# mjmyt/drone_path_planning_python

Measured on AMD Instinct MI355X. Metric: minimum-snap trajectories/sec (N drones × M segments, order 7) at 1/2/4/8 MI355X, higher is better.
Workload: dtype f64

## Files before the change

drone_path_planning_python_amd/csrc/msnap_collide.hip:

```cpp
#include <math.h>

#include "msnap_internal.h"
#include "msnap_collide.h"
#include "msnap_wave.h"

namespace msnap {


struct CollideGeom {
  int R, ro, Cn, S;
  int Rp;
  int os, oe;
  int sym;
  int n_rb;
  int upw;
  int upw_tail;
  long long split;
  int sparts;
  long long total;
  long long u_lo, u_n;
  int I_lo, I_hi;
  int part;
};

// ... 396 lines not shown
        bv[u] = e < nG * 6 ? cu.colbox[e] : 0.0;
      }
#pragma unroll
      for (int u = 0; u < kStageGroups * 6 / kSelThreads; ++u) {
        const int e = threadIdx.x + u * kSelThreads;
        if (e < nG * 6) sBox[e] = bv[u];
      }
    }
    __syncthreads();
  }
  auto load_box = [&](int gq, double(&B)[6]) {
#pragma unroll
    for (int k = 0; k < 6; ++k) {
      if constexpr (kStage) B[k] = sBox[gq * 6 + k];
      else B[k] = cu.colbox[(size_t)gq * 6 + k];
    }
  };
  if ((int)blockIdx.x >= n_rb) {
    constexpr int NW = kSelThreads / kWave, NS = kSelGroups * kSelTrips;
    __shared__ int gsum[NS * NW + 1];
    __shared__ int gbase, gtot;
    const int a0 = (blockIdx.x - n_rb) * kSelGroups, nG = (N + kColBlock - 1) / kColBlock;
    const int lane = threadIdx.x & (kWave - 1), w = threadIdx.x / kWave;
    unsigned long long kept = 0;
#pragma unroll
    for (int ai = 0; ai < kSelGroups; ++ai) {
      const int a = a0 + ai;
      double A[7], A6[6];
      load_box(a < nG ? a : nG - 1, A6);
#pragma unroll
      for (int k = 0; k < 6; ++k) A[k] = A6[k];
      A[6] = sCmax[a < nG ? a : nG - 1];
#pragma unroll
      for (int t = 0; t < kSelTrips; ++t) {
        bool keep = false;
        if (a + t * kSelThreads < nG) {
          const int b = a + t * kSelThreads + threadIdx.x, bc = b < nG ? b : nG - 1;
          double B6[6];
          load_box(bc, B6);
          const double lb2 = box_box_lb2(A, B6);
          keep = b < nG && (b == a || !((lb2 > A[6]) & (lb2 > sCmax[bc])));
        }
        const unsigned long long m = __ballot(keep);
        kept |= keep ? 1ull << (ai * kSelTrips + t) : 0ull;
        if (lane == 0) gsum[(ai * kSelTrips + t) * NW + w] = __popcll(m);
      }
    }
    __syncthreads();
    if (threadIdx.x < kWave) {
      int run = 0;
      for (int i0 = 0; i0 < NS * NW; i0 += kWave) {
        const int v = i0 + lane < NS * NW ? gsum[i0 + lane] : 0;
        int inc = v;
#pragma unroll
        for (int m = 1; m < kWave; m <<= 1) {
          const int o = __shfl_up(inc, m);
          inc += lane >= m ? o : 0;
        }
        if (i0 + lane < NS * NW) gsum[i0 + lane] = run + inc - v;
        run += __shfl(inc, kWave - 1);
      }
      if (lane == 0) {
        gbase = atomicAdd(&meta[kMetaGroups], run);
        gtot = run;
      }
    }
    __syncthreads();
    if (threadIdx.x < kSelGroups && a0 + (int)threadIdx.x < nG) {
      const int ai = threadIdx.x;
      const int s0 = gsum[ai * kSelTrips * NW], s1 = ai + 1 < kSelGroups ? gsum[(ai + 1) * kSelTrips * NW] : gtot;
      cg.astart[a0 + ai] = gbase + s0;
      cg.acnt[a0 + ai] = s1 - s0;
    }
#pragma unroll
    for (int ai = 0; ai < kSelGroups; ++ai)
#pragma unroll
      for (int t = 0; t < kSelTrips; ++t) {
        const bool keep = (kept >> (ai * kSelTrips + t)) & 1ull;
        const unsigned long long m = __ballot(keep);
        const int pos = gbase + gsum[(ai * kSelTrips + t) * NW + w] + __popcll(m & ((1ull << lane) - 1ull));
        if (keep && pos < cg.cap) {
          const int a = a0 + ai, b = a + t * kSelThreads + threadIdx.x;
          cg.glist[pos] = (a << 16) | b;
          if (b != a) cg.blist[(size_t)b * cg.nG + a] = pos + 1;
        }
      }
    return;
  }
  constexpr int GPB = kRowBlock / kColBlock;
  constexpr int NW = kSelThreads / kWave;
  __shared__ int wsum[kSelTrips][NW];
  __shared__ int sStart;
  __shared__ double sRow[GPB][8];
  __shared__ double sAll[8];
  const int I = blockIdx.x, lane = threadIdx.x & (kWave - 1), w = threadIdx.x / kWave;
  const int nsh = (N - I * kRowBlock + kColBlock - 1) / kColBlock;
  const int ng = nsh < GPB ? nsh : GPB;
  if (threadIdx.x < 7 * GPB) {
    const int q = threadIdx.x / 7, k = threadIdx.x % 7;
    if (q < ng) sRow[q][k] = k < 6 ? (kStage ? sBox[(I * GPB + q) * 6 + k] : cu.colbox[(size_t)(I * GPB + q) * 6 + k]) : sCmax[I * GPB + q];
  }
  __syncthreads();
  if (threadIdx.x < 7) {
    const int k = threadIdx.x;
    double v = sRow[0][k];
    for (int q = 1; q < ng; ++q) v = k < 3 ? fmin(v, sRow[q][k]) : fmax(v, sRow[q][k]);
    sAll[k] = v;
  }
  __syncthreads();
  unsigned long long mk[kSelTrips];
  bool keep[kSelTrips];
  double cbx[kSelTrips][6], cmx[kSelTrips];
#pragma unroll
  for (int t = 0; t < kSelTrips; ++t) {
    if (t * kSelThreads >= nsh) continue;
    const int k = t * kSelThreads + threadIdx.x, J = I * GPB + (k < nsh ? k : nsh - 1);
    load_box(J, cbx[t]);
    cmx[t] = sCmax[J];
  }
#pragma unroll
  for (int t = 0; t < kSelTrips; ++t) {
    const int k = t * kSelThreads + threadIdx.x;
    keep[t] = false;
    if (k < nsh) {
      keep[t] = true;
      if (k >= GPB) {
        const double cm = cmx[t];
        bool any = false;
        const double lb0 = box_box_lb2(sAll, cbx[t]);
        if (!((lb0 > sAll[6]) & (lb0 > cm))) {
          for (int q = 0; q < ng; ++q) {
            const double lb2 = box_box_lb2(sRow[q], cbx[t]);
            any |= !((lb2 > sRow[q][6]) & (lb2 > cm));
          }
        }
        keep[t] = any;
      }
    }
    mk[t] = __ballot(keep[t]);
    if (lane == 0) wsum[t][w] = __popcll(mk[t]);
  }
  __syncthreads();
  int all = 0, off[kSelTrips];
#pragma unroll
  for (int t = 0; t < kSelTrips; ++t) {
#pragma unroll
    for (int q = 0; q < NW; ++q) {
      if (q == w) off[t] = all;
      all += wsum[t][q];
    }
  }
  if (threadIdx.x == 0) {
    const int start = atomicAdd(&meta[kMetaTotal], all);
    sStart = start;
    meta[kMetaStart + I] = start;
    cnt[I] = all;
  }
  __syncthreads();
#pragma unroll
  for (int t = 0; t < kSelTrips; ++t)
    if (keep[t]) list[sStart + off[t] + __popcll(mk[t] & ((1ull << lane) - 1ull))] = (I << 16) | (t * kSelThreads + threadIdx.x);
}

__device__ __forceinline__ void
collide_span_list_body(const double *__restrict__ prow_t, const double *__restrict__ pcol, CollideGeom g,
                       double *__restrict__ part_d2, int32_t *__restrict__ part_j, double *__restrict__ cpart_d2,
                       int32_t *__restrict__ cpart_i, const int32_t *__restrict__ oid, const int32_t *__restrict__ list,
                       int sp_force, int slots, int32_t *__restrict__ meta) {
  constexpr int CB = kColBlock;
  __shared__ double sFold[CB * kWave];
  __shared__ int sFoldI[CB * kWave];
  const int lane = threadIdx.x;
  const int tot = meta[kMetaTotal];
  const CullSplit sp = cull_split(tot, slots, cull_nch(g.S), sp_force);
  if (blockIdx.x == 0 && lane == 0) {
    meta[kMetaParts] = sp.lo;
    meta[kMetaParts + 1] = sp.hi;
    meta[kMetaParts + 2] = sp.x;
  }
  const int items = sp.items(tot);
  const int xi = sp.x * sp.hi;
  auto share_of = [&](int it) { return it < xi ? it / sp.hi : sp.x + (it - xi) / sp.lo; };
  int it = blockIdx.x;
  int entry = it < items ? list[share_of(it)] : 0;
  while (it < items) {
    const int f = share_of(it);
    g.sparts = it < xi ? sp.hi : sp.lo;
    const int h = it - sp.item_of(f);
    const int I = entry >> 16, k = entry & 0xffff;
    const int nxt = it + gridDim.x;
    entry = nxt < items ? list[share_of(nxt)] : 0;
    const int crow = I * sp.hi + h;
    const int cj = I * kRowBlock + k * CB;
    const int ncols = g.Cn - cj < CB ? g.Cn - cj : CB;
    const bool two_sided = k >= kRowBlock / CB;
    RowSet rs;
#pragma unroll
    for (int rr = 0; rr < kRowsPerLane; ++rr) {
      const int raw = I * kRowBlock + rr * kWave + lane;
      rs.live[rr] = raw < g.R;
      rs.grow[rr] = rs.live[rr] ? raw : g.R - 1;
      rs.best[rr] = INFINITY;
      rs.bestj[rr] = -1;
    }
    const double *prowT = prow_t + (size_t)I * kRowBlock;
    if (ncols <= 2)
      collide_block<2, true>(g, prowT, pcol, cj, ncols, two_sided, rs, I, h, crow, lane, sFold, sFoldI, cpart_d2, cpart_i, oid);
    else if (ncols <= CB / 2)
      collide_block<CB / 2, true>(g, prowT, pcol, cj, ncols, two_sided, rs, I, h, crow, lane, sFold, sFoldI, cpart_d2, cpart_i, oid);
    else
      collide_block<CB, true>(g, prowT, pcol, cj, ncols, two_sided, rs, I, h, crow, lane, sFold, sFoldI, cpart_d2, cpart_i, oid);
#pragma unroll
    for (int rr = 0; rr < kRowsPerLane; ++rr) {
      part_d2[(size_t)it * kRowBlock + rr * kWave + lane] = rs.best[rr];
      part_j[(size_t)it * kRowBlock + rr * kWave + lane] = (rs.best[rr] == INFINITY) ? -1 : rs.bestj[rr];
    }
    it = nxt;
  }
}

constexpr int kGroupHalf = kColBlock / 2;
constexpr int kGroupLanes = kWave / 2;

constexpr int kFinishWaves = 4;
template <int kChunks>
__global__ void __launch_bounds__(kWave * kFinishWaves)
collide_finish_groups_kernel(int N, const int32_t *__restrict__ oid, const int32_t *__restrict__ meta, CullGroups cg,
                             double radius, double *__restrict__ min_dist, int32_t *__restrict__ partner,
                             int32_t *__restrict__ hit) {
  __shared__ int sItAll[kFinishWaves][kChunks * kWave];
  const int lane = threadIdx.x & (kWave - 1), w = __builtin_amdgcn_readfirstlane(threadIdx.x / kWave);
  int *sIt = sItAll[w];
  const int gq = blockIdx.x * kFinishWaves + w;
  if (gq >= cg.nG) return;
  int pl[kChunks];
#pragma unroll
  for (int c = 0; c < kChunks; ++c)
    pl[c] = (c * kWave < gq && c * kWave + lane < gq) ? cg.blist[(size_t)gq * cg.nG + c * kWave + lane] : 0;
  if (meta[kMetaGroups] > cg.cap) {
#pragma unroll
    for (int c = 0; c < kChunks; ++c)
      if (pl[c] > 0) cg.blist[(size_t)gq * cg.nG + c * kWave + lane] = 0;
    return;
  }
  const int nA = cg.acnt[gq], sA = cg.astart[gq];
  const int k = lane & (kColBlock - 1), e = lane >> 3;
  const int r = gq * kColBlock + k;
  const int out = r < N ? oid[r] : 0;
  int nB = 0;
#pragma unroll
  for (int c = 0; c < kChunks; ++c) {
    const unsigned long long m = __ballot(pl[c] > 0);
    if (pl[c] > 0) sIt[nB + __popcll(m & ((1ull << lane) - 1ull))] = pl[c] - 1;
    nB += __popcll(m);
  }
  __builtin_amdgcn_fence(__ATOMIC_RELEASE, "wavefront", "local");
  __builtin_amdgcn_wave_barrier();
  __builtin_amdgcn_fence(__ATOMIC_ACQUIRE, "wavefront", "local");
  double best = INFINITY;
  int bj = -1;
  constexpr int U = 8;
  for (int q0 = 0; q0 < nA + nB; q0 += U * (kWave / kColBlock)) {
    double d[U];
    int j[U];
#pragma unroll
    for (int u = 0; u < U; ++u) {
      const int q = q0 + u * (kWave / kColBlock) + e;
      d[u] = INFINITY;
      j[u] = -1;
      if (q < nA + nB) {
        const size_t slot = (q < nA ? (size_t)(sA + q) * 16 : (size_t)sIt[q - nA] * 16 + kColBlock) + k;
        d[u] = cg.cand_d2[slot];
        j[u] = cg.cand_j[slot];
      }
    }
#pragma unroll
    for (int u = 0; u < U; ++u)
      if (j[u] >= 0 && (bj < 0 || d[u] < best || (d[u] == best && j[u] < bj))) {
        best = d[u];
        bj = j[u];
      }
  }
#pragma unroll
  for (int m = kColBlock; m < kWave; m <<= 1) {
    const double o = shfl_xor_f64(best, m);
    const int oj = __shfl_xor(bj, m);
    if (oj >= 0 && (bj < 0 || o < best || (o == best && oj < bj))) {
      best = o;
      bj = oj;
    }
  }
  if (e == 0 && r < N) {
    const double dist = sqrt(bj >= 0 ? best : INFINITY);
    min_dist[out] = dist;
    partner[out] = bj;
    hit[out] = (dist < 2.0 * radius) ? 1 : 0;
  }
#pragma unroll
  for (int c = 0; c < kChunks; ++c)
    if (pl[c] > 0) cg.blist[(size_t)gq * cg.nG + c * kWave + lane] = 0;
}

constexpr int kGroupWaves = 4;
__global__ void __launch_bounds__(kWave, kGroupWaves)
collide_eval_groups_kernel(const double *__restrict__ pcol, int N, int S, const int32_t *__restrict__ oid,
                           const int32_t *__restrict__ meta, CullGroups cg, unsigned long long *__restrict__ hint) {
#pragma clang fp contract(off)
  const int lane = threadIdx.x;
  int tot = meta[kMetaGroups];
  if (blockIdx.x == 0 && lane == 0 && hint != nullptr)
    __hip_atomic_store(hint, cull_hint_pack(N, meta[kMetaTotal], tot), __ATOMIC_RELAXED, __HIP_MEMORY_SCOPE_SYSTEM);
  if (tot > cg.cap) tot = 0;
  const unsigned stride = (unsigned)S * 3u;
  const int per = (tot + 7) >> 3;
  auto item_of = [&](int v) { return (v >> 3) < per ? (v & 7) * per + (v >> 3) : tot; };
  int v = blockIdx.x, it = item_of(v);
  int entry = (it < tot && it < cg.cap) ? cg.glist[it] : 0;
  for (; (v >> 3) < per; v += gridDim.x, it = item_of(v)) {
    const int it_next = item_of(v + (int)gridDim.x);
    const int ent_raw = entry;
    entry = it_next < tot ? cg.glist[it_next] : 0;
    if (it >= tot) continue;
    const int ent = __builtin_amdgcn_readfirstlane(ent_raw);
    const int a = ent >> 16, b = ent & 0xffff;
    const bool diag = a == b;

    int lane_s = threadIdx.x;
    asm volatile("" : "+v"(lane_s));
    const int half = lane_s >> 5, ls = lane_s & (kGroupLanes - 1);
    double acc[kColBlock * kGroupHalf];
#pragma unroll
    for (int p = 0; p < kColBlock * kGroupHalf; ++p) acc[p] = INFINITY;
#pragma unroll 1
    for (int s0 = 0; s0 < S; s0 += kGroupLanes) {
      const int sq = s0 + ls < S ? s0 + ls : S - 1;
      const unsigned voff = (unsigned)sq * 24u;
      double cx[kGroupHalf], cy[kGroupHalf], cz[kGroupHalf];
#pragma unroll
      for (int c = 0; c < kGroupHalf; ++c) {
        const int d = b * kColBlock + half * kGroupHalf + c;
        const double *p = reinterpret_cast<const double *>(
            reinterpret_cast<const char *>(pcol + (size_t)(d < N ? d : N - 1) * stride) + (size_t)voff);
        cx[c] = p[0];
        cy[c] = p[1];
        cz[c] = p[2];
      }
      double rw[3][3];
      auto fetch = [&](int r, double(&dst)[3]) {
        const int d = a * kColBlock + r;
        const double *p = reinterpret_cast<const double *>(
            reinterpret_cast<const char *>(pcol + (size_t)(d < N ? d : N - 1) * stride) + (size_t)voff);
        dst[0] = p[0];
        dst[1] = p[1];
        dst[2] = p[2];
      };
      fetch(0, rw[0]);
      fetch(1, rw[1]);
#pragma unroll
      for (int r = 0; r < kColBlock; ++r) {
        if (r + 2 < kColBlock) fetch(r + 2, rw[(r + 2) % 3]);
        asm volatile("" ::: "memory");
        const double x = rw[r % 3][0], y = rw[r % 3][1], z = rw[r % 3][2];
#pragma unroll
        for (int c = 0; c < kGroupHalf; ++c) {
          const double dx = cx[c] - x, dy = cy[c] - y, dz = cz[c] - z;
          const double d2 = __builtin_fma(dz, dz, __builtin_fma(dy, dy, dx * dx));
          asm("v_min_f64 %0, %1, %0" : "+v"(acc[r * kGroupHalf + c]) : "v"(d2));
        }
      }
    }
#pragma unroll
    for (int n = 16, m = 16; n >= 1; n >>= 1, m >>= 1) {
      const bool up = (lane_s & m) != 0;
#pragma unroll
      for (int i = 0; i < n; ++i) {
        const double keep = up ? acc[i + n] : acc[i], send = up ? acc[i] : acc[i + n];
        acc[i] = __builtin_fmin(keep, __shfl_xor(send, m));
      }
    }
    double v = acc[0];
    int lane_c = threadIdx.x;
    asm volatile("" : "+v"(lane_c));
    const int pr = (lane_c & (kGroupLanes - 1)) >> 2, pc = lane_c & (kGroupHalf - 1), half_c = lane_c >> 5;
    const int ra = a * kColBlock + pr, cb = b * kColBlock + half_c * kGroupHalf + pc;
    const int oi = oid[ra < N ? ra : N - 1], oj = oid[cb < N ? cb : N - 1];
    if (ra >= N || cb >= N || (diag && ra == cb)) v = INFINITY;
    {
      double w = v;
      int wj = oj;
#pragma unroll
      for (int m = 1; m <= 32; m = (m == 2 ? 32 : m << 1)) {
        const double o = __shfl_xor(w, m);
        const int ojx = __shfl_xor(wj, m);
        const bool take = (o < w) | ((o == w) & (ojx < wj));
        w = take ? o : w;
        wj = take ? ojx : wj;
      }
      if ((lane & 35) == 0) {
        cg.cand_d2[(size_t)it * 16 + pr] = w;
        cg.cand_j[(size_t)it * 16 + pr] = w < INFINITY ? wj : -1;
      }
    }
    {
      double w = v;
      int wi = oi;
#pragma unroll
      for (int m = 4; m <= 16; m <<= 1) {
        const double o = __shfl_xor(w, m);
        const int oix = __shfl_xor(wi, m);
        const bool take = (o < w) | ((o == w) & (oix < wi));
        w = take ? o : w;
        wi = take ? oix : wi;
      }
      if ((lane_c & (kGroupLanes - 1)) < kGroupHalf) {
        const int k = kColBlock + half_c * kGroupHalf + pc;
        cg.cand_d2[(size_t)it * 16 + k] = w;
        cg.cand_j[(size_t)it * 16 + k] = (!diag && w < INFINITY) ? wi : -1;
      }
    }
  }
}

__global__ void __launch_bounds__(kWave, 4)
collide_eval_shares_kernel(const double *__restrict__ prow_t, const double *__restrict__ pcol, CollideGeom g,
                           double *__restrict__ part_d2, int32_t *__restrict__ part_j, double *__restrict__ cpart_d2,
                           int32_t *__restrict__ cpart_i, const int32_t *__restrict__ oid, const int32_t *__restrict__ list,
                           int sp_force, int slots, int32_t *__restrict__ meta, unsigned long long *__restrict__ hint,
                           int groups_cap) {
  if (groups_cap > 0 && meta[kMetaGroups] <= groups_cap) return;
  if (blockIdx.x == 0 && threadIdx.x == 0 && hint != nullptr)
    __hip_atomic_store(hint, cull_hint_pack(g.R, meta[kMetaTotal], meta[kMetaGroups]), __ATOMIC_RELAXED,
                       __HIP_MEMORY_SCOPE_SYSTEM);
  collide_span_list_body(prow_t, pcol, g, part_d2, part_j, cpart_d2, cpart_i, oid, list, sp_force, slots, meta);
}

__global__ void __launch_bounds__(kWave)
collide_short_kernel(const double *__restrict__ prow, const double *__restrict__ pcol, int R, int ro, int Cn, int S,
                     double radius, double *__restrict__ min_dist, int32_t *__restrict__ partner,
                     int32_t *__restrict__ hit, int raw) {
#pragma clang fp contract(off)
  const int r = blockIdx.x * kWave + threadIdx.x;
  if (r >= R) return;
  const int grow = ro + r;
  const double *pr = prow + (size_t)r * S * 3;
  double best = INFINITY;
  int bestj = -1;
  for (int j = 0; j < Cn; ++j) {
    const double *pc = pcol + (size_t)j * S * 3;
    double m = INFINITY;
    for (int sq = 0; sq < S; ++sq) {
      const double dx = pc[(size_t)sq * 3 + 0] - pr[(size_t)sq * 3 + 0];
      const double dy = pc[(size_t)sq * 3 + 1] - pr[(size_t)sq * 3 + 1];
      const double dz = pc[(size_t)sq * 3 + 2] - pr[(size_t)sq * 3 + 2];
      const double d2 = __builtin_fma(dz, dz, __builtin_fma(dy, dy, dx * dx));
      m = __builtin_fmin(d2, m);
    }
    if (j == grow) m = INFINITY;
    if (m < best) {
      best = m;
      bestj = j;
    }
  }
  if (raw) {
    min_dist[r] = best;
    partner[r] = (best == INFINITY) ? -1 : bestj;
    return;
  }
  const double dist = sqrt(best);
  min_dist[r] = dist;
  partner[r] = (best == INFINITY) ? -1 : bestj;
  hit[r] = (dist < 2.0 * radius) ? 1 : 0;
}

constexpr int kMergeRows = 16;
constexpr int kMergeParts = 16;
__global__ void __launch_bounds__(kMergeRows * kMergeParts)
collide_merge_kernel(const double *__restrict__ part_d2, const int32_t *__restrict__ part_j, CollideGeom g,
                     const double *__restrict__ cpart_d2, const int32_t *__restrict__ cpart_i, double radius,
                     double *__restrict__ min_dist, int32_t *__restrict__ partner, int32_t *__restrict__ hit,
                     const int32_t *__restrict__ oid, const int32_t *__restrict__ cnt, const int32_t *__restrict__ meta,
                     int groups_cap = 0) {
  if (groups_cap > 0 && meta[kMetaGroups] <= groups_cap) return;
  __shared__ double sD[kMergeParts][kMergeRows];
  __shared__ int sJ[kMergeParts][kMergeRows];
  const int lr = threadIdx.x & (kMergeRows - 1), q = threadIdx.x / kMergeRows;
  const int r_raw = blockIdx.x * kMergeRows + lr;
  const int r = r_raw < g.R ? r_raw : g.R - 1;
  const int out = oid ? oid[r] : r;
  double best = INFINITY;
  int bj = -1;
  constexpr int U = 8;
  auto sweep = [&](const double *pd, const int32_t *pj, size_t pitch, int n) {
    for (int s0 = q; s0 < n; s0 += U * kMergeParts) {
      double v[U];
      int j[U];
#pragma unroll
      for (int k = 0; k < U; ++k) {
        const int sidx = s0 + k * kMergeParts;
        const int sc = sidx < n ? sidx : n - 1;
        v[k] = pd[(size_t)sc * pitch];
        j[k] = sidx < n ? pj[(size_t)sc * pitch] : -1;
      }
#pragma unroll
      for (int k = 0; k < U; ++k) {
        if (j[k] >= 0 && (v[k] < best || (v[k] == best && j[k] < bj))) {
          best = v[k];
          bj = j[k];
        }
      }
    }
  };
  if (cnt) {
    const int I = __builtin_amdgcn_readfirstlane(r / kRowBlock);
    CullSplit sp;
    sp.lo = meta[kMetaParts];
    sp.hi = meta[kMetaParts + 1];
    sp.x = meta[kMetaParts + 2];
    const int f0 = meta[kMetaStart + I], first_item = sp.item_of(f0), n_items = sp.item_of(f0 + cnt[I]) - first_item;
    const size_t first = (size_t)first_item * kRowBlock + (r - I * kRowBlock);
    sweep(part_d2 + first, part_j + first, kRowBlock, n_items);
    if (I > 0) sweep(cpart_d2 + r, cpart_i + r, (size_t)g.R, I * sp.hi);
  } else if (g.total > 0) {
    const int I = r / kRowBlock;
    long long ua = collide_ustart(g, I), ub = collide_ustart(g, I + 1) - 1;
    ua = ua < g.u_lo ? g.u_lo : ua;
    ub = ub >= g.u_lo + g.u_n ? g.u_lo + g.u_n - 1 : ub;
    if (ub >= ua) {
      const long long wf = collide_share_of(g, ua), wl = collide_share_of(g, ub);
      const size_t first = ((size_t)wf + (I - g.I_lo)) * g.sparts * kRowBlock + (r - I * kRowBlock);
      sweep(part_d2 + first, part_j + first, kRowBlock, (int)(wl - wf + 1) * g.sparts);
    }
    const int Ib = I < g.I_hi + 1 ? I : g.I_hi + 1;
    if (g.sym && Ib > g.I_lo) sweep(cpart_d2 + r, cpart_i + r, (size_t)g.R, (Ib - g.I_lo) * g.sparts);
  }
  sD[q][lr] = best;
  sJ[q][lr] = bj;
  __syncthreads();
  if (q == 0 && r_raw < g.R) {
#pragma unroll
    for (int k = 1; k < kMergeParts; ++k) {
      const double v = sD[k][lr];
      const int j = sJ[k][lr];
      if (j >= 0 && (v < best || (v == best && j < bj))) {
        best = v;
        bj = j;
      }
    }
    if (g.part) {
      min_dist[r] = best;
      partner[r] = bj;
    } else {
      const double dist = sqrt(best);
      min_dist[out] = dist;
      partner[out] = bj;
      hit[out] = (dist < 2.0 * radius) ? 1 : 0;
    }
  }
}

__global__ void __launch_bounds__(256)
collide_finish_kernel(const unsigned char *__restrict__ parts, size_t part_stride, int n_parts, int N, int row_offset,
                      int n_rows, double radius, double *__restrict__ min_dist, int32_t *__restrict__ partner,
                      int32_t *__restrict__ hit) {
  const int i = blockIdx.x * 256 + threadIdx.x;
  if (i >= n_rows) return;
  const int r = row_offset + i;
  double best = INFINITY;
  int bj = -1;
  for (int p = 0; p < n_parts; ++p) {
    const unsigned char *base = parts + (size_t)p * part_stride;
    const double v = reinterpret_cast<const double *>(base)[r];
    const int j = reinterpret_cast<const int32_t *>(base + (size_t)N * sizeof(double))[r];
    if (j >= 0 && (v < best || (v == best && j < bj))) {
      best = v;
      bj = j;
    }
  }
  const double dist = sqrt(best);
  min_dist[i] = dist;
  partner[i] = bj;
  hit[i] = (dist < 2.0 * radius) ? 1 : 0;
}

__global__ void __launch_bounds__(256) collide_part_clear_kernel(double *__restrict__ d2, int32_t *__restrict__ pj, int N) {
  const int i = blockIdx.x * 256 + threadIdx.x;
  if (i < N) {
    d2[i] = INFINITY;
    pj[i] = -1;
  }
}


__global__ void __launch_bounds__(kWave * kKeyDrones)
collide_key_kernel(const double *__restrict__ pos, int N, int S, double *__restrict__ box, unsigned *__restrict__ key) {
  const int lane = threadIdx.x & (kWave - 1);
  const int d = blockIdx.x * kKeyDrones + __builtin_amdgcn_readfirstlane(threadIdx.x / kWave);
  if (d >= N) return;
  const double *p = pos + (size_t)d * S * 3;
  double lo[3] = {INFINITY, INFINITY, INFINITY}, hi[3] = {-INFINITY, -INFINITY, -INFINITY};
  const int E = S * 3;
  for (int e0 = 0; e0 < E; e0 += 3 * kWave) {
#pragma unroll
    for (int q = 0; q < 3; ++q) {
      const int e = e0 + q * kWave + lane;
      const double v = e < E ? p[e] : __builtin_nan("");
      const int k = (lane + q) % 3;
      if (__builtin_isfinite(v)) {
#pragma unroll
        for (int kk = 0; kk < 3; ++kk)
          if (k == kk) {
            lo[kk] = v < lo[kk] ? v : lo[kk];
            hi[kk] = v > hi[kk] ? v : hi[kk];
          }
      }
    }
  }
#pragma unroll
  for (int k = 0; k < 3; ++k) {
    lo[k] = uniform_f64(wave_minmax_f64<false>(lo[k]));
    hi[k] = uniform_f64(wave_minmax_f64<true>(hi[k]));
  }
  if (lane < 3) {
    box[(size_t)d * 6 + lane] = lane == 0 ? lo[0] : lane == 1 ? lo[1] : lo[2];
    box[(size_t)d * 6 + 3 + lane] = lane == 0 ? hi[0] : lane == 1 ? hi[1] : hi[2];
  }
  if (lane == 0) key[d] = drone_sort_key(lo, hi);
}

constexpr int kRankWaves = 16;
constexpr int kRankTile = 16;
template <int kRankKeys>
__global__ void __launch_bounds__(kWave * kRankWaves)
collide_rank_kernel(const unsigned *__restrict__ key, int N, int32_t *__restrict__ perm, const double *__restrict__ box,
                    unsigned long long *__restrict__ bound, int32_t *__restrict__ zero, int n_zero,
                    int32_t *__restrict__ meta) {
  __shared__ int cnt[kRankWaves][kRankTile];
  {
    const int gid = blockIdx.x * (kWave * kRankWaves) + threadIdx.x;
    uniform_for<int>(threadIdx.x, n_zero, gridDim.x * (kWave * kRankWaves), [&](int z) { zero[z] = 0; },
                     blockIdx.x * (kWave * kRankWaves));
    if (gid == 0) {
      meta[kMetaTotal] = 0;
      meta[kMetaGroups] = 0;
    }
  }
  const int lane = threadIdx.x & (kWave - 1), w = __builtin_amdgcn_readfirstlane(threadIdx.x / kWave);
  const int nq = (N + kRankWaves * kWave - 1) / (kRankWaves * kWave);
  const int i0 = blockIdx.x * kRankTile;
  unsigned kraw[kRankKeys];
#pragma unroll
  for (int q = 0; q < kRankKeys; ++q) {
    const int j = (w * nq + q) * kWave + lane;
    kraw[q] = key[(q < nq && j < N) ? j : 0];
  }
  const unsigned ktile = key[i0 + (lane & (kRankTile - 1)) < N ? i0 + (lane & (kRankTile - 1)) : N - 1];
  double bx[6] = {0.0, 0.0, 0.0, 0.0, 0.0, 0.0};
  if (threadIdx.x < kRankTile && i0 + (int)threadIdx.x < N) {
#pragma unroll
    for (int k = 0; k < 6; ++k) bx[k] = box[(size_t)(i0 + threadIdx.x) * 6 + k];
  }
  unsigned long long mine[kRankKeys];
#pragma unroll
  for (int q = 0; q < kRankKeys; ++q) {
    const int j = (w * nq + q) * kWave + lane;
    mine[q] = (q < nq && j < N) ? ((unsigned long long)kraw[q] << 32) | (unsigned)j : ~0ull;
  }
#pragma unroll
  for (int t = 0; t < kRankTile; ++t) {
    const int i = i0 + t < N ? i0 + t : N - 1;
    const unsigned long long ki = ((unsigned long long)(unsigned)__builtin_amdgcn_readlane((int)ktile, t) << 32) | (unsigned)i;
    int c = 0;
#pragma unroll
    for (int q = 0; q < kRankKeys; ++q)
      if (q < nq) c += __popcll(__ballot(mine[q] < ki));
    if (lane == 0) cnt[w][t] = c;
  }
  lds_barrier();
  if (threadIdx.x < kRankTile && i0 + (int)threadIdx.x < N) {
    int r = 0;
#pragma unroll
    for (int q = 0; q < kRankWaves; ++q) r += cnt[q][threadIdx.x];
    const int i = i0 + threadIdx.x;
    perm[r] = i;
    const bool has = (bx[0] <= bx[3]) & (bx[1] <= bx[4]) & (bx[2] <= bx[5]);
    bound[r] = has ? 0x7ff0000000000000ull : 0ull;
  }
}

#ifndef MSNAP_TILE_E
#define MSNAP_TILE_E 15
#endif
constexpr int kTileE = MSNAP_TILE_E, kTileRows = 64, kTileHalo = 4;
constexpr int kTilePitch = kTileE + 1 + (kTileE & 1);
static_assert(kTileE % 3 == 0, "whole samples per tile");
constexpr int kBoxGroups = 32;
__global__ void __launch_bounds__(256)
collide_gather_kernel(const double *__restrict__ pos, int N, int Rp, int E, double *__restrict__ prow_t,
                      double *__restrict__ psorted, const int32_t *__restrict__ perm, unsigned long long *__restrict__ bound,
                      const double *__restrict__ box, double *__restrict__ colbox, int nx, int ny, int n_box,
                      int32_t *__restrict__ fill, size_t fill_n) {
#pragma clang fp contract(off)
  __shared__ double tile[(kTileRows + kTileHalo) * kTilePitch];
  __shared__ double sF[kTileHalo][kTileRows];
  const int tid = threadIdx.x;
  const int nb = (int)blockIdx.x - nx * ny;
  if (nb >= n_box) {
    const size_t stride = (size_t)(gridDim.x - nx * ny - n_box) * 256;
    uniform_for<size_t>(tid, fill_n, stride, [&](size_t i) { fill[i] = -1; }, (size_t)(nb - n_box) * 256);
    return;
  }
  if (nb >= 0) {
    const int gq = nb * kBoxGroups + (tid >> 3), r = gq * kColBlock + (tid & 7);
    double g6[6];
#pragma unroll
    for (int k = 0; k < 6; ++k) g6[k] = k < 3 ? INFINITY : -INFINITY;
    if (r < N) {
      const double *bx = box + (size_t)perm[r] * 6;
#pragma unroll
      for (int k = 0; k < 6; ++k) g6[k] = bx[k];
    }
#pragma unroll
    for (int k = 0; k < 6; ++k) {
      auto fold = [k](double a, double c) { return k < 3 ? fmin(a, c) : fmax(a, c); };
      g6[k] = fold(g6[k], dpp_f64<0xB1>(g6[k]));
// ... 434 lines not shown
```

drone_path_planning_python_amd/csrc/msnap_wave.h:

```cpp
#pragma once

#include <hip/hip_runtime.h>

namespace msnap {

__device__ __forceinline__ double shfl_xor_f64(double v, int mask) {
  const int lo = __shfl_xor(__double2loint(v), mask);
  const int hi = __shfl_xor(__double2hiint(v), mask);
  return __hiloint2double(hi, lo);
}

template <int CTRL>
__device__ __forceinline__ double dpp_f64(double v) {
  const int lo = __builtin_amdgcn_mov_dpp(__double2loint(v), CTRL, 0xF, 0xF, true);
  const int hi = __builtin_amdgcn_mov_dpp(__double2hiint(v), CTRL, 0xF, 0xF, true);
  return __hiloint2double(hi, lo);
}
template <bool MAX>
__device__ __forceinline__ double wave_minmax_f64(double v) {
  auto fold = [](double a, double b) { return MAX ? ((b > a) ? b : a) : ((b < a) ? b : a); };
  v = fold(v, dpp_f64<0xB1>(v));
  v = fold(v, dpp_f64<0x4E>(v));
  v = fold(v, dpp_f64<0x141>(v));
  v = fold(v, dpp_f64<0x140>(v));
  v = fold(v, __shfl_xor(v, 16));
  v = fold(v, __shfl_xor(v, 32));
  return v;
}
__device__ __forceinline__ double wave_min_f64(double v) { return wave_minmax_f64<false>(v); }
__device__ __forceinline__ double wave_max_f64(double v) { return wave_minmax_f64<true>(v); }
template <bool MAX>
__device__ __forceinline__ double wave_minmax_num_f64(double v) {
  auto fold = [](double a, double b) { return MAX ? __builtin_fmax(a, b) : __builtin_fmin(a, b); };
  v = fold(v, dpp_f64<0xB1>(v));
  v = fold(v, dpp_f64<0x4E>(v));
  v = fold(v, dpp_f64<0x141>(v));
  v = fold(v, dpp_f64<0x140>(v));
  v = fold(v, __shfl_xor(v, 16));
  v = fold(v, __shfl_xor(v, 32));
  return v;
}

template <class I, class Body>
__device__ __forceinline__ void uniform_for(I first, I count, I stride, Body &&body, I base = 0) {
  for (I e0 = base; e0 < count; e0 += stride) {
    const I e = e0 + first;
    if (e < count) body(e);
  }
}

__device__ __forceinline__ double uniform_f64(double v) {
  return __hiloint2double(__builtin_amdgcn_readfirstlane(__double2hiint(v)),
                          __builtin_amdgcn_readfirstlane(__double2loint(v)));
}

}
```

Before: 60.45 million.

## Interleave group-kernel lane mapping and reduce with permlane swaps

Reassigns lanes in the group collision kernel so the two column halves are interleaved on odd and even lanes. A branch-free address select picks each lane's column drone. The first two transpose-reduction stages now use permlane32/permlane16 swap instructions instead of cross-lane shuffles, and the later stages use explicit v_min_f64. The candidate-reduction masks and store predicates are rewritten to match the new lane layout. It also adds an optional compile-time timeline probe, and the interleaving changes the memory access pattern of the column loads.

```diff
diff --git a/drone_path_planning_python_amd/csrc/msnap_collide.hip b/drone_path_planning_python_amd/csrc/msnap_collide.hip
--- a/drone_path_planning_python_amd/csrc/msnap_collide.hip
+++ b/drone_path_planning_python_amd/csrc/msnap_collide.hip
@@ -722,6 +722,17 @@
 }
 
 constexpr int kGroupWaves = 4;
+#ifdef MSNAP_TOOLS_TIMELINE
+constexpr int kGroupTimelineRows = 8192;
+__device__ unsigned long long g_groups_timeline[kGroupTimelineRows * 8];
+#define MSNAP_GTL(k)                                                                                 \
+  do {                                                                                               \
+    if (threadIdx.x == 0 && tl_item < 2 && blockIdx.x * 2 + tl_item < (unsigned)kGroupTimelineRows)  \
+      g_groups_timeline[(blockIdx.x * 2 + tl_item) * 8 + (k)] = wall_clock64();                      \
+  } while (0)
+#else
+#define MSNAP_GTL(k) do { } while (0)
+#endif
 __global__ void __launch_bounds__(kWave, kGroupWaves)
 collide_eval_groups_kernel(const double *__restrict__ pcol, int N, int S, const int32_t *__restrict__ oid,
                            const int32_t *__restrict__ meta, CullGroups cg, unsigned long long *__restrict__ hint) {
@@ -741,13 +752,18 @@
     const int ent_raw = entry;
     entry = it_next < tot ? cg.glist[it_next] : 0;
     if (it >= tot) continue;
+#ifdef MSNAP_TOOLS_TIMELINE
+    const unsigned tl_item = (unsigned)(v - (int)blockIdx.x) / gridDim.x;
+#endif
+    MSNAP_GTL(0);
     const int ent = __builtin_amdgcn_readfirstlane(ent_raw);
     const int a = ent >> 16, b = ent & 0xffff;
     const bool diag = a == b;
 
     int lane_s = threadIdx.x;
     asm volatile("" : "+v"(lane_s));
-    const int half = lane_s >> 5, ls = lane_s & (kGroupLanes - 1);
+    const int ls = lane_s >> 1;
+    const unsigned hsel = 0u - (unsigned)(lane_s & 1);
     double acc[kColBlock * kGroupHalf];
 #pragma unroll
     for (int p = 0; p < kColBlock * kGroupHalf; ++p) acc[p] = INFINITY;
@@ -758,9 +774,11 @@
       double cx[kGroupHalf], cy[kGroupHalf], cz[kGroupHalf];
 #pragma unroll
       for (int c = 0; c < kGroupHalf; ++c) {
-        const int d = b * kColBlock + half * kGroupHalf + c;
+        const int d0 = b * kColBlock + c, d1 = d0 + kGroupHalf;
+        const int e0 = d0 < N ? d0 : N - 1, e1 = d1 < N ? d1 : N - 1;
+        const unsigned step = (unsigned)(e1 - e0) * stride * 8u;
         const double *p = reinterpret_cast<const double *>(
-            reinterpret_cast<const char *>(pcol + (size_t)(d < N ? d : N - 1) * stride) + (size_t)voff);
+            reinterpret_cast<const char *>(pcol + (size_t)e0 * stride) + (size_t)(voff + (hsel & step)));
         cx[c] = p[0];
         cy[c] = p[1];
         cz[c] = p[2];
@@ -788,35 +806,45 @@
           asm("v_min_f64 %0, %1, %0" : "+v"(acc[r * kGroupHalf + c]) : "v"(d2));
         }
       }
-    }
-#pragma unroll
-    for (int n = 16, m = 16; n >= 1; n >>= 1, m >>= 1) {
-      const bool up = (lane_s & m) != 0;
+      if (s0 < 3 * kGroupLanes) MSNAP_GTL(1 + s0 / kGroupLanes);
+    }
+    MSNAP_GTL(4);
+    int lane_c = threadIdx.x;
+    asm volatile("" : "+v"(lane_c));
+    const int pr = lane_c >> 3, pc = (lane_c >> 1) & (kGroupHalf - 1), half_c = lane_c & 1;
+    const int ra = a * kColBlock + pr, cb = b * kColBlock + half_c * kGroupHalf + pc;
+    const int oi = oid[ra < N ? ra : N - 1], oj = oid[cb < N ? cb : N - 1];
+    asm volatile("" ::: "memory");
+#pragma unroll
+    for (int i = 0; i < 16; ++i) swap_min_f64<32>(acc[i], acc[i + 16]);
+#pragma unroll
+    for (int i = 0; i < 8; ++i) swap_min_f64<16>(acc[i], acc[i + 8]);
+#pragma unroll
+    for (int n = 4, m = 8; n >= 1; n >>= 1, m >>= 1) {
+      const bool up = (lane_c & m) != 0;
 #pragma unroll
       for (int i = 0; i < n; ++i) {
         const double keep = up ? acc[i + n] : acc[i], send = up ? acc[i] : acc[i + n];
-        acc[i] = __builtin_fmin(keep, __shfl_xor(send, m));
-      }
-    }
+        const double got = shfl_xor_f64(send, m);
+        acc[i] = keep;
+        asm("v_min_f64 %0, %1, %0" : "+v"(acc[i]) : "v"(got));
+      }
+    }
+    MSNAP_GTL(5);
     double v = acc[0];
-    int lane_c = threadIdx.x;
-    asm volatile("" : "+v"(lane_c));
-    const int pr = (lane_c & (kGroupLanes - 1)) >> 2, pc = lane_c & (kGroupHalf - 1), half_c = lane_c >> 5;
-    const int ra = a * kColBlock + pr, cb = b * kColBlock + half_c * kGroupHalf + pc;
-    const int oi = oid[ra < N ? ra : N - 1], oj = oid[cb < N ? cb : N - 1];
     if (ra >= N || cb >= N || (diag && ra == cb)) v = INFINITY;
     {
       double w = v;
       int wj = oj;
 #pragma unroll
-      for (int m = 1; m <= 32; m = (m == 2 ? 32 : m << 1)) {
+      for (int m = 1; m <= 4; m <<= 1) {
         const double o = __shfl_xor(w, m);
         const int ojx = __shfl_xor(wj, m);
         const bool take = (o < w) | ((o == w) & (ojx < wj));
         w = take ? o : w;
         wj = take ? ojx : wj;
       }
-      if ((lane & 35) == 0) {
+      if ((lane_c & 7) == 0) {
         cg.cand_d2[(size_t)it * 16 + pr] = w;
         cg.cand_j[(size_t)it * 16 + pr] = w < INFINITY ? wj : -1;
       }
@@ -825,21 +853,28 @@
       double w = v;
       int wi = oi;
 #pragma unroll
-      for (int m = 4; m <= 16; m <<= 1) {
+      for (int m = 8; m <= 32; m <<= 1) {
         const double o = __shfl_xor(w, m);
         const int oix = __shfl_xor(wi, m);
         const bool take = (o < w) | ((o == w) & (oix < wi));
         w = take ? o : w;
         wi = take ? oix : wi;
       }
-      if ((lane_c & (kGroupLanes - 1)) < kGroupHalf) {
+      if (lane_c < kColBlock) {
         const int k = kColBlock + half_c * kGroupHalf + pc;
         cg.cand_d2[(size_t)it * 16 + k] = w;
         cg.cand_j[(size_t)it * 16 + k] = (!diag && w < INFINITY) ? wi : -1;
       }
     }
-  }
-}
+    MSNAP_GTL(6);
+  }
+}
+#ifdef MSNAP_TOOLS_TIMELINE
+extern "C" int msnap_debug_read_groups_timeline(unsigned long long *out, int n_words) {
+  if (hipDeviceSynchronize() != hipSuccess) return MSNAP_EHIP;
+  return hipMemcpyFromSymbol(out, HIP_SYMBOL(g_groups_timeline), (size_t)n_words * 8) == hipSuccess ? MSNAP_OK : MSNAP_EHIP;
+}
+#endif
 
 __global__ void __launch_bounds__(kWave, 4)
 collide_eval_shares_kernel(const double *__restrict__ prow_t, const double *__restrict__ pcol, CollideGeom g,
diff --git a/drone_path_planning_python_amd/csrc/msnap_wave.h b/drone_path_planning_python_amd/csrc/msnap_wave.h
--- a/drone_path_planning_python_amd/csrc/msnap_wave.h
+++ b/drone_path_planning_python_amd/csrc/msnap_wave.h
@@ -8,6 +8,25 @@
   const int lo = __shfl_xor(__double2loint(v), mask);
   const int hi = __shfl_xor(__double2hiint(v), mask);
   return __hiloint2double(hi, lo);
+}
+
+template <int ROW>
+__device__ __forceinline__ void swap_min_f64(double &a, double b) {
+  static_assert(ROW == 16 || ROW == 32, "the lane swaps exist for rows of 16 and of 32 lanes");
+  typedef unsigned u32x2 __attribute__((ext_vector_type(2)));
+  const unsigned alo = (unsigned)__double2loint(a), ahi = (unsigned)__double2hiint(a);
+  const unsigned blo = (unsigned)__double2loint(b), bhi = (unsigned)__double2hiint(b);
+  u32x2 lo, hi;
+  if constexpr (ROW == 32) {
+    lo = __builtin_amdgcn_permlane32_swap(alo, blo, false, false);
+    hi = __builtin_amdgcn_permlane32_swap(ahi, bhi, false, false);
+  } else {
+    lo = __builtin_amdgcn_permlane16_swap(alo, blo, false, false);
+    hi = __builtin_amdgcn_permlane16_swap(ahi, bhi, false, false);
+  }
+  a = __hiloint2double((int)hi[0], (int)lo[0]);
+  const double o = __hiloint2double((int)hi[1], (int)lo[1]);
+  asm("v_min_f64 %0, %1, %0" : "+v"(a) : "v"(o));
 }
 
 template <int CTRL>
```

Measured after the change: 60.44 million, median of 2. No clear change (-0.0%).
